# semchan/DCT_Pruning

Measured on AMD Instinct MI355X. Metric: feature-map DCT+score throughput, higher is better.
Workload: dtype f32; 1 GPU; resnet_50 hooked feature maps (49 tensors, 22720 maps/sample: 56x56 x1344, 28x28 x3200, 14x14 x9472, 7x7 x8704), batch 256, limit=steps; global_batch=256, launch_mode=one launch per tile shape, units_rank0=49

## Files before the change

### dct_pruning_amd/csrc/api.hip

```cpp
#include <hip/hip_runtime.h>
#include <stdint.h>

#include <initializer_list>
#include <mutex>

#include "../../include/dctscore.h"
#include "dcts_internal.h"
#include "grid_caps.h"
#include "rect.h"
#ifdef DCTS_FUSED_STAMPS
#include "split_common.hpp"
#endif

using namespace dctsi;

namespace {

struct TensorView {
  const float* x;
  int64_t N, C_total, H, W, strideN, strideC, strideH, strideW;
  int32_t c_begin, c_count;
  bool pad_front_if_odd;

  int pad() const { return (pad_front_if_odd && (H % 2 != 0)) ? 1 : 0; }
// ... 113 lines not shown
    if (algo == DCTS_ALGO_TILE2D || algo == DCTS_ALGO_FUSED) {
      if (!tile_shape || !aligned16) return kUnsupported;
      if (algo == DCTS_ALGO_TILE2D) return {HP == 224 ? Family::Tile2d : Family::Tile2g, DCTS_OK};
      return {has_fused2(HP) ? Family::Fused2 : Family::Fused, DCTS_OK};
    }
    return {Family::Direct, DCTS_OK};
  }
  const bool split_ok = tile_shape && aligned16;
  if (algo == DCTS_ALGO_SPLIT && !split_ok) return kUnsupported;
  if (algo == DCTS_ALGO_AUTO || algo == DCTS_ALGO_FUSED || algo == DCTS_ALGO_PIPE || algo == DCTS_ALGO_TILE2D) {
    if (tile_shape)
      for (const auto& t : kTileOrder) {
        const Family f = t.fam;
        if ((algo != DCTS_ALGO_AUTO && algo != t.algo) || !serves(f, HP)) continue;
        if (!aligned16 && traits(f).base16) continue;
        if (f == Family::Tile2g && algo == DCTS_ALGO_AUTO && aligned16 && tile2g_loses(HP)) continue;
        return {f, DCTS_OK};
      }
    if (pad == 1 && v.dense_maps() && (algo == DCTS_ALGO_AUTO || algo == DCTS_ALGO_TILE2D) && has_tile2g_pad(HP))
      return {Family::Tile2gPad, DCTS_OK};
    if (algo != DCTS_ALGO_AUTO) return kUnsupported;
  }
  if (split_ok && algo != DCTS_ALGO_DIRECT) return {Family::Split, DCTS_OK};
  return {Family::Direct, DCTS_OK};
}

TileBatch single_batch(const TensorView& v, float* out) { return single_tensor_batch(v.base(), out, v.nmaps(), v.strideC); }

struct BasisSlot {
  uintptr_t lo, hi;
  void* ws;
  void* stream;
  int HP, WP;
};
constexpr int kBasisSlots = 16;
BasisSlot g_basis[kBasisSlots] = {};
int g_basis_next = 0;
std::mutex g_basis_mu;

bool basis_cached(void* ws, void* stream, int HP, int WP) {
  std::lock_guard<std::mutex> lk(g_basis_mu);
  for (const BasisSlot& b : g_basis)
    if (b.hi && b.ws == ws && b.stream == stream && b.HP == HP && b.WP == WP) return true;
  return false;
}
void basis_forget_range(const void* p, size_t bytes) {
  if (!p || !bytes) return;
  const uintptr_t lo = reinterpret_cast<uintptr_t>(p), hi = lo + bytes;
  std::lock_guard<std::mutex> lk(g_basis_mu);
  for (BasisSlot& b : g_basis)
    if (b.hi && b.lo < hi && lo < b.hi) b = BasisSlot{};
}
void basis_forget(void* ws) {
  if (!ws) return;
  const uintptr_t a = reinterpret_cast<uintptr_t>(ws);
  std::lock_guard<std::mutex> lk(g_basis_mu);
  for (BasisSlot& b : g_basis)
    if (b.hi && (b.ws == ws || (b.lo <= a && a < b.hi))) b = BasisSlot{};
}
void basis_remember(void* ws, const void* tables, size_t table_bytes, void* stream, int HP, int WP) {
  const uintptr_t lo = reinterpret_cast<uintptr_t>(tables), hi = lo + table_bytes;
  std::lock_guard<std::mutex> lk(g_basis_mu);
  for (BasisSlot& b : g_basis)
    if (b.hi && (b.ws == ws || (b.lo < hi && lo < b.hi))) b = BasisSlot{};
  g_basis[g_basis_next] = BasisSlot{lo, hi, ws, stream, HP, WP};
  g_basis_next = (g_basis_next + 1) % kBasisSlots;
}

int run(bool store, const TensorView& v, float* out, void* workspace, size_t workspace_bytes, void* stream, int32_t algo,
        bool cache_basis = true) {
  if (const int rc = validate(v, {out}, Checks::All)) return rc;
  const Choice c = choose(v, algo, store, v.aligned16());
  if (c.err) return c.err;
  const int HP = (int)v.HP(), WP = (int)v.WP(), pad = v.pad();
  const MapGeom g = map_geom(v);
  hipStream_t st = reinterpret_cast<hipStream_t>(stream);
  switch (c.fam) {
    case Family::Rect: return dispatch_rect(rect_geom(v), out, store ? 1 : 0, st);
    case Family::CodeletDma: return dispatch_codelet_dma(HP, g, out, st);
    case Family::Codelet: return dispatch_codelet(store ? 1 : 0, HP, WP, pad, g, out, st);
    case Family::Direct: break;
    case Family::Lane: {
      MultiGeom mg;
      for (int i = 0; i < kMultiItems; ++i) mg.it[i] = MultiItem{g, out, 0};
      mg.total_groups = (g.nmaps + 63) / 64;
      mg.count = 1;
      return dispatch_lane(HP, mg, st);
    }
    case Family::Split: {
      const SplitWs sws = split_ws(g.nmaps, HP);
      if (!workspace || workspace_bytes < sws.total) return DCTS_E_WORKSPACE;
      if (reinterpret_cast<uintptr_t>(workspace) & 15) return DCTS_E_ALIGN;
      basis_forget_range(workspace, sws.total);
      return dispatch_split(HP, g, out, workspace, st);
    }
    default: {
      if (!store) return traits(c.fam).batch(HP, single_batch(v, out), st);
      const long long tile_bytes = (long long)HP * WP * 4;
      const long long ws_maps = workspace ? (long long)(workspace_bytes / (size_t)tile_bytes) : 0;
      if (ws_maps < 1 || (reinterpret_cast<uintptr_t>(workspace) & 15)) return DCTS_E_WORKSPACE;
      float* scratch = reinterpret_cast<float*>(workspace);
      basis_forget_range(workspace, workspace_bytes);
      switch (c.fam) {
        case Family::Tile2d: return dispatch_tile2d_coeff(HP, v.base(), g.nmaps, out, scratch, ws_maps, st);
        case Family::Tile2g: return dispatch_tile2g_coeff(HP, v.base(), g.nmaps, out, scratch, ws_maps, st);
        case Family::Fused2: return dispatch_fused2_coeff(HP, v.base(), g.nmaps, out, scratch, ws_maps, st);
        default: return dispatch_fused_coeff(HP, v.base(), g.nmaps, out, scratch, ws_maps, st);
      }
    }
  }

  const DirectWs ws = direct_ws(g.nmaps, HP, WP);
  if (!workspace) return ws.total ? DCTS_E_WORKSPACE : DCTS_E_NULL;
  if (workspace_bytes < ws.total) return DCTS_E_WORKSPACE;
  char* wsp = reinterpret_cast<char*>(workspace);
  float* CHt = reinterpret_cast<float*>(wsp + ws.off_ch);
  float* CWt = reinterpret_cast<float*>(wsp + ws.off_cw);
  float* T = reinterpret_cast<float*>(wsp + ws.off_t);
  int rc_tables = 0;
  if (!cache_basis || !basis_cached(workspace, stream, HP, WP)) {
    basis_forget_range(workspace, ws.total);
    const int rc = launch_basis(CHt, HP, CWt, WP, st);
    if (cache_basis && rc == hipSuccess) basis_remember(workspace, wsp + ws.off_ch, ws.off_t - ws.off_ch, stream, HP, WP);
    if (!cache_basis) rc_tables = rc;
  } else {
    basis_forget_range(wsp + ws.off_t, ws.total - ws.off_t);
  }
  const int rc = dispatch_direct(store ? 1 : 0, pad, g, ws.grid, CHt, CWt, T, out, st);
  return rc ? rc : rc_tables;
}

int coeff_algo(const TensorView& v) {
  const int HP = (int)v.HP();
  if (v.pad() != 0 || !v.dense_square() || (v.strideN * 4) % 16 != 0 || !v.aligned16()) return DCTS_ALGO_AUTO;
  if (serves(Family::Tile2d, HP) || serves(Family::Tile2g, HP)) return DCTS_ALGO_TILE2D;
  if (serves(Family::Fused, HP) || serves(Family::Fused2, HP)) return DCTS_ALGO_FUSED;
  return DCTS_ALGO_AUTO;
}

template <class F>
int for_chunks(int64_t N, int64_t c_count, long long chunk, bool whole_samples, F f) {
  if (whole_samples) {
    const int64_t ns = chunk / c_count;
    for (int64_t n0 = 0; n0 < N; n0 += ns)
      if (const int rc = f(n0, (N - n0) < ns ? (N - n0) : ns, (int64_t)0, c_count)) return rc;
    return DCTS_OK;
  }
  for (int64_t n = 0; n < N; ++n)
    for (int64_t c0 = 0; c0 < c_count; c0 += chunk)
      if (const int rc = f(n, (int64_t)1, c0, (c_count - c0) < chunk ? (c_count - c0) : chunk)) return rc;
  return DCTS_OK;
}

struct CoeffWs {
  long long chunk;
  float* coeff;
  void* inner;
  size_t inner_bytes;
};
CoeffWs coeff_ws(void* workspace, size_t workspace_bytes, long long chunk, size_t tile) {
  const size_t off_inner = align_up((size_t)chunk * tile, 256);
  char* wsp = reinterpret_cast<char*>(workspace);
  return CoeffWs{chunk, reinterpret_cast<float*>(wsp), wsp + off_inner, workspace_bytes - off_inner};
}

template <class Reduce>
int coeff_chunks(const TensorView& v, const CoeffWs& w, bool whole_samples, int algo, void* workspace, size_t workspace_bytes,
                 void* stream, Reduce reduce) {
  basis_forget(workspace);
  basis_forget_range(workspace, workspace_bytes);
// ... 296 lines not shown

int dcts_has_half_kernel(int64_t H, int64_t W) { return has_half(H, W) ? 1 : 0; }

int dcts_energy_typed(const void* x, int32_t dtype, int64_t N, int64_t C_total, int64_t H, int64_t W, int64_t strideN,
                      int64_t strideC, int64_t strideH, int64_t strideW, int32_t c_begin, int32_t c_count,
                      int32_t pad_front_if_odd, float* out_nc, void* workspace, size_t workspace_bytes, void* stream) {
  if (dtype == DCTS_DTYPE_F32)
    return dcts_energy_f32(reinterpret_cast<const float*>(x), N, C_total, H, W, strideN, strideC, strideH, strideW, c_begin,
                           c_count, pad_front_if_odd, out_nc, workspace, workspace_bytes, stream);
  if (!is_half_dtype(dtype)) return DCTS_E_UNSUPPORTED;
  const TensorView v = view_of(x, N, C_total, H, W, strideN, strideC, strideH, strideW, c_begin, c_count, pad_front_if_odd);
  if (const int rc = validate(v, {out_nc}, Checks::All, true, elem_mask(dtype))) return rc;
  hipStream_t st = reinterpret_cast<hipStream_t>(stream);
  const uint16_t* xh = reinterpret_cast<const uint16_t*>(x);
  if (has_half(H, W) && v.pad() == 0 && strideH == W)
    return dispatch_half((int)H, dtype, HalfGeom{xh, v.nmaps(), strideN, strideC, c_count, c_begin, v.contiguous() ? 1 : 0}, out_nc, st);

  if (!workspace) return DCTS_E_WORKSPACE;
  if (reinterpret_cast<uintptr_t>(workspace) & 15) return DCTS_E_ALIGN;
  const size_t map = (size_t)H * W * 4;
  const size_t inner_bytes = align_up(dcts_workspace_bytes(N, c_count, H, W), 256);
  if (workspace_bytes < inner_bytes + map) return DCTS_E_WORKSPACE;
  long long chunk = (long long)((workspace_bytes - inner_bytes) / map);
  if ((size_t)chunk * map > kHalfStageCap && kHalfStageCap >= map) chunk = (long long)(kHalfStageCap / map);
  float* stage = reinterpret_cast<float*>(reinterpret_cast<char*>(workspace) + inner_bytes);
  void* inner = inner_bytes ? workspace : nullptr;
  basis_forget_range(stage, (size_t)chunk * map);
  return for_chunks(N, c_count, chunk, chunk >= c_count, [&](int64_t n0, int64_t ns, int64_t c0, int64_t nc) -> int {
    const HalfGeom g{xh + n0 * strideN, ns * nc, strideN, strideC, (int)nc, (int)(c_begin + c0), (ns == 1 || strideN == nc * strideC) ? 1 : 0};
    if (const int rc = launch_upcast_half(dtype, g, (int)H, (int)W, strideH, stage, st)) return rc;
    const TensorView s{stage, ns, nc, H, W, nc * H * W, H * W, W, 1, 0, (int32_t)nc, pad_front_if_odd != 0};
    return run(false, s, out_nc + n0 * c_count + c0, inner, inner_bytes, stream, DCTS_ALGO_AUTO);
  });
}

int dcts_has_nhwc_kernel(int64_t H, int64_t W) { return has_nhwc(H, W) ? 1 : 0; }

size_t dcts_nhwc_workspace_bytes(int32_t, int64_t, int64_t, int64_t, int64_t) { return 0; }

int dcts_energy_nhwc(const void* x, int32_t dtype, int64_t N, int64_t C_total, int64_t H, int64_t W, int64_t strideN,
                     int64_t strideH, int64_t strideW, int32_t c_begin, int32_t c_count, float* out_nc, void*, size_t, void* stream) {
  if (dtype != DCTS_DTYPE_F32 && !is_half_dtype(dtype)) return DCTS_E_UNSUPPORTED;
  const TensorView v = view_of(x, N, C_total, H, W, strideN, 1, strideH, strideW, c_begin, c_count, 0);
  if (const int rc = validate(v, {out_nc}, Checks::All, true, elem_mask(dtype), true)) return rc;
  if (!has_nhwc(H, W)) return DCTS_E_UNSUPPORTED;
  return dispatch_nhwc((int)H, dtype, NhwcGeom{x, N, strideN, strideH, strideW, c_begin, c_count}, out_nc, reinterpret_cast<hipStream_t>(stream));
}

int dcts_batch_sum_f32(const float* energy_nc, int64_t N, int64_t C_count, float* out_c,
                       void* stream) {
  if (!energy_nc || !out_c) return DCTS_E_NULL;
  if (N <= 0 || C_count <= 0) return DCTS_E_SHAPE;
  return launch_batch_sum(energy_nc, N, C_count, out_c, reinterpret_cast<hipStream_t>(stream));
}

int dcts_running_mean_update_f32(const float* energy_nc, int64_t N, int64_t C_count,
                                 float* feature_result, float total_before, void* stream) {
  if (!energy_nc || !feature_result) return DCTS_E_NULL;
  if (N <= 0 || C_count <= 0) return DCTS_E_SHAPE;
  return launch_running_mean(energy_nc, N, C_count, feature_result, total_before, reinterpret_cast<hipStream_t>(stream));
}

int dcts_energy_multi_f32(const dcts_tensor_item* items, int32_t count, int64_t H, int64_t W,
                          int32_t pad_front_if_odd, void* workspace, size_t workspace_bytes, void* stream) {
  if (!items) return DCTS_E_NULL;
  if (count <= 0 || H <= 0 || W <= 0) return DCTS_E_SHAPE;
  for (int32_t i = 0; i < count; ++i)
    if (const int rc = validate(view_of(items[i], H, W, pad_front_if_odd), {items[i].out_nc}, Checks::Align)) return rc;
  const TensorView v0 = view_of(items[0], H, W, pad_front_if_odd);
  const int HP = (int)v0.HP(), WP = (int)v0.WP(), pad = v0.pad();
  hipStream_t st = reinterpret_cast<hipStream_t>(stream);
  if (has_codelet(HP, WP)) {
    const int G = codelet_group_size(HP);
    for (int32_t i0 = 0; i0 < count; i0 += kMultiItems) {
      const int n = (count - i0) < kMultiItems ? (count - i0) : kMultiItems;
      MultiGeom mg;
      long long groups = 0;
      for (int i = 0; i < n; ++i) {
        mg.it[i].g = map_geom(view_of(items[i0 + i], H, W, pad_front_if_odd));
        mg.it[i].out = items[i0 + i].out_nc;
        mg.it[i].group_begin = groups;
        groups += (mg.it[i].g.nmaps + G - 1) / G;
      }
      for (int i = n; i < kMultiItems; ++i) mg.it[i] = mg.it[0];
      mg.total_groups = groups;
      mg.count = n;
      const int rc = dispatch_codelet_multi(HP, pad, mg, st);
      if (rc) return rc;
    }
    return DCTS_OK;
  }
  TileBatch tb;
  Family fam = Family::Direct;
  int nb = 0;
  auto flush = [&]() -> int {
    if (!nb) return DCTS_OK;
    for (int i = nb; i < kTileItems; ++i) {
      tb.x[i] = tb.x[0];
      tb.out[i] = tb.out[0];
      tb.begin[i + 1] = tb.begin[nb];
    }
    tb.map_elems = H * W;
    tb.total = tb.begin[nb];
    tb.count = nb;
    nb = 0;
    return traits(fam).batch(HP, tb, st);
  };
  for (int32_t i = 0; i < count; ++i) {
    const TensorView v = view_of(items[i], H, W, pad_front_if_odd);
    const Choice c = choose(v, DCTS_ALGO_AUTO, false, true);
    if (!c.err && traits(c.fam).batch && (v.aligned16() || !traits(c.fam).base16)) {
      if (nb == 0) tb.begin[0] = 0;
      fam = c.fam;
      tb.x[nb] = v.base();
      tb.out[nb] = items[i].out_nc;
      tb.begin[nb + 1] = tb.begin[nb] + v.nmaps();
      if (++nb == kTileItems) {
        const int rc = flush();
        if (rc) return rc;
      }
      continue;
    }
    const int rc = run(false, v, items[i].out_nc, workspace, workspace_bytes, stream, DCTS_ALGO_AUTO);
    if (rc) return rc;
  }
  return flush();
}

int dcts_energy_mixed_f32(const dcts_shaped_item* items, int32_t count, void* workspace, size_t workspace_bytes,
                          void* stream) {
  if (!items) return DCTS_E_NULL;
  if (count <= 0) return DCTS_E_SHAPE;
  hipStream_t st = reinterpret_cast<hipStream_t>(stream);
  for (int32_t i = 0; i < count; ++i)
    if (const int rc = validate(view_of(items[i]), {items[i].t.out_nc}, Checks::Align)) return rc;
  auto eligible = [&](const dcts_shaped_item& it) {
    return it.H == it.W && mixed_has((int)it.H) && !(it.pad_front_if_odd && (it.H % 2 != 0));
  };
  MixedGeom mg;
  int n = 0;
  long long groups = 0;
  auto flush = [&]() -> int {
    if (!n) return DCTS_OK;
    for (int i = n; i < kMixedItems; ++i) mg.it[i] = mg.it[0];
    mg.total_groups = groups;
    mg.count = n;
    n = 0;
    groups = 0;
    return dispatch_codelet_mixed(mg, st);
  };
  for (int32_t i = 0; i < count; ++i) {
    if (!eligible(items[i])) continue;
    mg.it[n].g = map_geom(view_of(items[i]));
    mg.it[n].out = items[i].t.out_nc;
    mg.it[n].group_begin = groups;
    const int G = 64 / (int)items[i].H;
    groups += (mg.it[n].g.nmaps + G - 1) / G;
    if (++n == kMixedItems) {
      const int rc = flush();
      if (rc) return rc;
    }
  }
  int rc = flush();
  if (rc) return rc;
  dcts_tensor_item buf[64];
  for (int32_t i = 0; i < count; ++i) {
    if (eligible(items[i])) continue;
    bool seen = false;
    for (int32_t k = 0; k < i && !seen; ++k)
      seen = !eligible(items[k]) && items[k].H == items[i].H && items[k].W == items[i].W &&
// ... 58 lines not shown
```

### dct_pruning_amd/csrc/codelet.hip

```cpp
#include <hip/hip_runtime.h>
#include <stdint.h>

#include "../../include/dctscore.h"
#include "codelet_schedule.hpp"
#include "codelet_sizes.h"
#include "dct_codelets.hpp"
#include "dcts_internal.h"
#include "grid_caps.h"
#include "split_roles.hpp"

using namespace dctsi;

namespace {

template <int O0, int O1, int O2, int O3>
__device__ __forceinline__ void lds_write_addtid4(unsigned base, float a, float b, float c, float d) {
  static_assert(O3 < 65536 && O0 >= 0, "16-bit offset field");
  asm volatile(
      "s_mov_b32 m0, %0\n\ts_nop 0\n\t"
      "ds_write_addtid_b32 %1 offset:%5\n\tds_write_addtid_b32 %2 offset:%6\n\t"
      "ds_write_addtid_b32 %3 offset:%7\n\tds_write_addtid_b32 %4 offset:%8"
      :
      : "s"(base), "v"(a), "v"(b), "v"(c), "v"(d), "n"(O0), "n"(O1), "n"(O2), "n"(O3)
      : "memory", "m0");
// ... 29 lines not shown
      dcts::static_for<HP>([&](auto i) DCTS_LAMBDA_INLINE { xr[decltype(i)::value] = 0.f; });
    }
  }
  float y[HP];
  dcts::Dct2<HP>::run(xr, y);
  y[0] *= dcts::kInvSqrt2;
  if constexpr (G == 1 && HP % 4 == 0) {
    if (act1) {
      const unsigned base = (unsigned)__builtin_amdgcn_readfirstlane((int)(unsigned)(unsigned long long)(lds_ptr)my);
      dcts::static_for<HP / 4>([&](auto i) DCTS_LAMBDA_INLINE {
        constexpr int k0 = 4 * decltype(i)::value;
        lds_write_addtid4<k0 * S * 4, (k0 + 1) * S * 4, (k0 + 2) * S * 4, (k0 + 3) * S * 4>(base, y[k0], y[k0 + 1], y[k0 + 2], y[k0 + 3]);
      });
    }
  } else
  if (act1) {
    float* dst = my + g1 * MAP_LDS + c;
    dcts::static_for<HP>([&](auto i) DCTS_LAMBDA_INLINE {
      constexpr int kk = decltype(i)::value;
      dst[kk * S] = y[kk];
    });
  }
  wave_fence();

  float z[WP], w[WP];
  {
    const float* src = my + (act2 ? g2 : 0) * MAP_LDS + (act2 ? k : 0) * S;
    dcts::static_for<WP>([&](auto i) DCTS_LAMBDA_INLINE {
      constexpr int cc = decltype(i)::value;
      z[cc] = src[cc];
    });
  }
  dcts::Dct2<WP>::run(z, w);
  w[0] *= dcts::kInvSqrt2;
  const long long m2 = grp * G + g2;
  if constexpr (STORE_COEFF) {
    if (act2 && m2 < g.nmaps) {
      constexpr float sc = float(2.0 / dcts::cx_sqrt(double(HP) * double(WP)));
      float* o = out + (m2 * HP + k) * WP;
      dcts::static_for<WP>([&](auto i) DCTS_LAMBDA_INLINE {
        constexpr int l = decltype(i)::value;
        o[l] = w[l] * sc;
      });
    }
  } else {
    float e = 0.f;
    dcts::static_for<WP>([&](auto i) DCTS_LAMBDA_INLINE {
      constexpr int l = decltype(i)::value;
      e = fmaf(w[l], w[l], e);
    });
    if (!act2) e = 0.f;
    DCTS_MAP_SUM(HP, e, k)
    if (act2 && k == 0 && m2 < g.nmaps) {
      constexpr float sc = float(4.0 / (double(HP) * double(WP)));
      out[m2] = e * sc;
    }
  }
  wave_fence();
}

template <int HP, int WP, int PAD, bool STORE_COEFF>
__global__ __launch_bounds__((64 * CodeletCfg<HP>::WAVES)) void k_energy_codelet(
    MapGeom g, float* __restrict__ out) {
  using Cfg = CodeletCfg<HP>;
  constexpr int G = Cfg::G, WAVES = Cfg::WAVES;
  __shared__ float slab[WAVES][Cfg::WAVE_LDS];

  const int lane = threadIdx.x & 63;
  const int wave = threadIdx.x >> 6;
  float* my = slab[wave];

  const int g1 = lane / WP, c = lane - g1 * WP;
  const int g2 = lane / HP, k = lane - g2 * HP;
  const bool act1 = g1 < G, act2 = g2 < G;

  const long long ngroups = (g.nmaps + G - 1) / G;
  const long long wave_gid = (long long)blockIdx.x * WAVES + wave;
  const long long nwaves = (long long)gridDim.x * WAVES;

  for (long long grp = wave_gid; grp < ngroups; grp += nwaves)
    codelet_group<HP, WP, PAD, STORE_COEFF>(g, out, grp, my, g1, c, g2, k, act1, act2);
}

template <int HP, int WP, int PAD>
__global__ __launch_bounds__((64 * CodeletCfg<HP>::WAVES)) void k_energy_codelet_multi(MultiGeom mg) {
  using Cfg = CodeletCfg<HP>;
  constexpr int G = Cfg::G, WAVES = Cfg::WAVES;
  __shared__ float slab[WAVES][Cfg::WAVE_LDS];

  const int lane = threadIdx.x & 63;
  const int wave = threadIdx.x >> 6;
  float* my = slab[wave];
  const int g1 = lane / WP, c = lane - g1 * WP;
  const int g2 = lane / HP, k = lane - g2 * HP;
  const bool act1 = g1 < G, act2 = g2 < G;

  const long long wave_gid = (long long)blockIdx.x * WAVES + wave;
  const long long nwaves = (long long)gridDim.x * WAVES;
  int t = 0;
  for (long long grp = wave_gid; grp < mg.total_groups; grp += nwaves) {
    while (t + 1 < mg.count && grp >= mg.it[t + 1].group_begin) ++t;
    t = __builtin_amdgcn_readfirstlane(t);
    const MultiItem& item = mg.it[t];
    codelet_group<HP, WP, PAD, false>(item.g, item.out, grp - item.group_begin, my, g1, c, g2, k, act1, act2);
  }
}

constexpr int mixed_slab_floats() {
  int m = 0;
#define DCTS_CASE(N) \
  if (CodeletCfg<N>::WAVE_LDS > m) m = CodeletCfg<N>::WAVE_LDS;
  DCTS_MIXED_SIZES(DCTS_CASE)
#undef DCTS_CASE
  return m;
}

template <int E>
__device__ __forceinline__ void mixed_group(const MultiItem& item, long long grp, float* my, int lane) {
  using Cfg = CodeletCfg<E>;
  const int g1 = lane / E, c = lane - g1 * E;
  const bool act = g1 < Cfg::G;
  codelet_group<E, E, 0, false>(item.g, item.out, grp, my, g1, c, g1, c, act, act);
}

__global__ __launch_bounds__((64 * kMixedWaves)) void k_energy_codelet_mixed(MixedGeom mg) {
  __shared__ float slab[kMixedWaves][mixed_slab_floats()];
  const int lane = threadIdx.x & 63;
  const int wave = threadIdx.x >> 6;
  float* my = slab[wave];
  const long long wave_gid = (long long)blockIdx.x * kMixedWaves + wave;
  const long long nwaves = (long long)gridDim.x * kMixedWaves;
  int t = 0;
  for (long long grp = wave_gid; grp < mg.total_groups; grp += nwaves) {
    while (t + 1 < mg.count && grp >= mg.it[t + 1].group_begin) ++t;
    t = __builtin_amdgcn_readfirstlane(t);
    const MultiItem& item = mg.it[t];
    const long long local = grp - item.group_begin;
    switch (__builtin_amdgcn_readfirstlane(item.g.H)) {
#define DCTS_CASE(N)                          \
  case N:                                     \
    mixed_group<N>(item, local, my, lane);    \
    break;
      DCTS_MIXED_SIZES(DCTS_CASE)
#undef DCTS_CASE
      default:
        break;
    }
  }
}

template <int N>
struct LaneCfg {
  static constexpr int NN = N * N;
  static constexpr int G = kLaneMultiGroup;
  static constexpr int SLAB = (G * NN + 3) / 4 * 4;
  static constexpr int ITERS = (G * NN / 4 + 63) / 64;
  static constexpr int WAVES = kLaneMultiWaves;
  static_assert(NN % 2 == 1, "lane stride must be odd (bank conflicts) - even tiles use the codelet kernel");
};

struct LaneGroup {
  const float* src;
  float* out;
  long long m0;
  int nm;
  int dense;
  int item;
};

template <int N>
__device__ __forceinline__ void lane_stage(const LaneGroup& gr, lds_ptr my, int lane) {
  using Cfg = LaneCfg<N>;
  if (!gr.dense) return;
  const int nfl = gr.nm * Cfg::NN, nq = nfl >> 2, rem = nfl & 3;
  const unsigned long long sa = reinterpret_cast<unsigned long long>(gr.src);
  const unsigned long long src = ((unsigned long long)__builtin_amdgcn_readfirstlane((int)(sa >> 32)) << 32) |
                                 (unsigned)__builtin_amdgcn_readfirstlane((int)sa);
  const unsigned base = (unsigned)__builtin_amdgcn_readfirstlane((int)(unsigned)(unsigned long long)my);
#pragma unroll
  for (int it = 0; it < Cfg::ITERS; ++it) {
    const int q = it * 64 + lane;
    if (q < nq) {
      const unsigned dst = base + it * 1024;
      const unsigned off = (unsigned)q * 16u;
      asm volatile("s_mov_b32 m0, %0\n\ts_nop 0\n\tglobal_load_lds_dwordx4 %1, %2"
                   :
                   : "s"(dst), "v"(off), "s"(src)
                   : "memory", "m0");
    }
  }
  if (lane < rem) my[4 * nq + lane] = gr.src[4 * nq + lane];
}

template <int N>
__device__ __forceinline__ void lane_compute(const MapGeom& g, const LaneGroup& gr, lds_ptr my, int lane,
                                             float (&v)[N * N]) {
  constexpr int NN = N * N;
  const bool act = lane < gr.nm;
  if (gr.dense) {
    lds_cptr p = my + (act ? lane : 0) * NN;
    dcts::static_for<NN>([&](auto i) DCTS_LAMBDA_INLINE { v[decltype(i)::value] = p[decltype(i)::value]; });
  } else {
    const float* p = map_base(g, gr.m0 + (act ? lane : 0));
    dcts::static_for<NN>([&](auto i) DCTS_LAMBDA_INLINE { v[decltype(i)::value] = p[decltype(i)::value]; });
  }
}

template <int N>
__device__ __forceinline__ float lane_energy(float (&v)[N * N]) {
  dcts::static_for<N>([&](auto ic) DCTS_LAMBDA_INLINE {
    constexpr int c = decltype(ic)::value;
    float in[N], o[N];
    dcts::static_for<N>([&](auto ir) DCTS_LAMBDA_INLINE { in[decltype(ir)::value] = v[decltype(ir)::value * N + c]; });
    dcts::Dct2<N>::run(in, o);
    o[0] *= dcts::kInvSqrt2;
    dcts::static_for<N>([&](auto ir) DCTS_LAMBDA_INLINE { v[decltype(ir)::value * N + c] = o[decltype(ir)::value]; });
  });
  float e = 0.f;
  dcts::static_for<N>([&](auto ir) DCTS_LAMBDA_INLINE {
    constexpr int r = decltype(ir)::value;
    float in[N], o[N];
    dcts::static_for<N>([&](auto ic) DCTS_LAMBDA_INLINE { in[decltype(ic)::value] = v[r * N + decltype(ic)::value]; });
    dcts::Dct2<N>::run(in, o);
    o[0] *= dcts::kInvSqrt2;
    dcts::static_for<N>([&](auto ic) DCTS_LAMBDA_INLINE { e = fmaf(o[decltype(ic)::value], o[decltype(ic)::value], e); });
  });
  constexpr float sc = float(4.0 / (double(N) * double(N)));
  return e * sc;
}

__device__ __forceinline__ LaneGroup lane_group_of(const MapGeom& g, float* out, long long grp, int nn, int item) {
  LaneGroup gr;
  gr.m0 = grp * 64;
  const long long left = g.nmaps - gr.m0;
  gr.nm = (int)(left < 64 ? left : 64);
  gr.src = g.x + (long long)g.c_begin * g.strideC + gr.m0 * nn;
  gr.dense = (g.contiguous && g.strideC == nn && ((reinterpret_cast<unsigned long long>(gr.src) & 15) == 0)) ? 1 : 0;
  gr.out = out + gr.m0;
  gr.item = item;
  return gr;
}

template <int N>
__global__ __launch_bounds__((64 * LaneCfg<N>::WAVES)) void k_energy_lane_multi(MultiGeom mg) {
  using Cfg = LaneCfg<N>;
  __shared__ __attribute__((aligned(16))) float slab[Cfg::WAVES][Cfg::SLAB];
  const int lane = threadIdx.x & 63;
  const int wave = threadIdx.x >> 6;
  const lds_ptr my = (lds_ptr)slab[wave];
  const long long wave_gid = (long long)blockIdx.x * Cfg::WAVES + wave;
  const long long nwaves = (long long)gridDim.x * Cfg::WAVES;
  int t = 0;
  auto locate = [&](long long grp) DCTS_LAMBDA_INLINE {
    while (t + 1 < mg.count && grp >= mg.it[t + 1].group_begin) ++t;
    t = __builtin_amdgcn_readfirstlane(t);
    return lane_group_of(mg.it[t].g, mg.it[t].out, grp - mg.it[t].group_begin, Cfg::NN, t);
  };
  if (wave_gid >= mg.total_groups) return;
  LaneGroup cur = locate(wave_gid);
  lane_stage<N>(cur, my, lane);
  for (long long grp = wave_gid; grp < mg.total_groups; grp += nwaves) {
    asm volatile("s_waitcnt vmcnt(0)" ::: "memory");
    float v[Cfg::NN];
    lane_compute<N>(mg.it[cur.item].g, cur, my, lane, v);
    asm volatile("s_waitcnt lgkmcnt(0)" ::: "memory");
    const LaneGroup done = cur;
    if (grp + nwaves < mg.total_groups) {
      cur = locate(grp + nwaves);
      lane_stage<N>(cur, my, lane);
    }
    const float e = lane_energy<N>(v);
    if (lane < done.nm) done.out[lane] = e;
  }
}

template <int N>
__global__ __launch_bounds__((64 * CodeletCfg<N>::WAVES)) void k_energy_codelet_dma(
    MapGeom g, float* __restrict__ out) {
  using Cfg = CodeletCfg<N>;
  constexpr int G = Cfg::G, S = Cfg::S, MAP_LDS = Cfg::MAP_LDS, WAVES = Cfg::WAVES;
  constexpr int NN = N * N;
  constexpr int QPG = G * NN / 4;
  constexpr int DMA_IT = (QPG + 63) / 64;
  constexpr int SLAB = ((Cfg::WAVE_LDS > DMA_IT * 256 ? Cfg::WAVE_LDS : DMA_IT * 256) + 3) / 4 * 4;
  static_assert((G * NN) % 4 == 0, "group must be a whole number of 16-byte quads");
  __shared__ __attribute__((aligned(16))) float slab[WAVES][SLAB];

  const int lane = threadIdx.x & 63;
  const int wave = threadIdx.x >> 6;
  float* my = slab[wave];
  const int g1 = lane / N, c = lane - g1 * N;
  const bool act = g1 < G;

  const long long ngroups = (g.nmaps + G - 1) / G;
  const long long wave_gid = (long long)blockIdx.x * WAVES + wave;
  const long long nwaves = (long long)gridDim.x * WAVES;
  const float* x0 = g.x + (long long)g.c_begin * g.strideC;

  auto prefetch = [&](long long grp) DCTS_LAMBDA_INLINE {
    const long long m0 = grp * G;
    const long long left = g.nmaps - m0;
    const int nq = (int)((left < G ? left : G) * (NN / 4));
    const float* src = x0 + m0 * NN;
#pragma unroll
    for (int it = 0; it < DMA_IT; ++it) {
      const int q = it * 64 + lane;
      if (q < nq)
        __builtin_amdgcn_global_load_lds((const __attribute__((address_space(1))) void*)(src + 4 * q),
                                         (__attribute__((address_space(3))) void*)(my + it * 256), 16, 0, 0);
    }
  };

  if (wave_gid < ngroups) prefetch(wave_gid);
  for (long long grp = wave_gid; grp < ngroups; grp += nwaves) {
    asm volatile("s_waitcnt vmcnt(0)" ::: "memory");
    const long long m1 = grp * G + g1;
    const bool valid = act && m1 < g.nmaps;
    float xr[N], y[N];
    {
      const float* src = my + (valid ? g1 * NN + c : 0);
      dcts::static_for<N>([&](auto i) DCTS_LAMBDA_INLINE {
        constexpr int r = decltype(i)::value;
        xr[r] = src[r * N];
      });
      if (!valid) dcts::static_for<N>([&](auto i) DCTS_LAMBDA_INLINE { xr[decltype(i)::value] = 0.f; });
    }
    dcts::Dct2<N>::run(xr, y);
    y[0] *= dcts::kInvSqrt2;
    __builtin_amdgcn_fence(__ATOMIC_RELEASE, "wavefront");
    __builtin_amdgcn_wave_barrier();
    if (act) {
      float* dst = my + g1 * MAP_LDS + c;
      dcts::static_for<N>([&](auto i) DCTS_LAMBDA_INLINE {
        constexpr int kk = decltype(i)::value;
        dst[kk * S] = y[kk];
      });
    }
    wave_fence();
    float z[N], w[N];
    {
      const float* src = my + (act ? g1 : 0) * MAP_LDS + (act ? c : 0) * S;
      dcts::static_for<N>([&](auto i) DCTS_LAMBDA_INLINE {
        constexpr int cc = decltype(i)::value;
        z[cc] = src[cc];
      });
    }
    asm volatile("s_waitcnt lgkmcnt(0)" ::: "memory");
    __builtin_amdgcn_fence(__ATOMIC_RELEASE, "wavefront");
    __builtin_amdgcn_wave_barrier();
    if (grp + nwaves < ngroups) prefetch(grp + nwaves);
    dcts::Dct2<N>::run(z, w);
    w[0] *= dcts::kInvSqrt2;
    float e = 0.f;
    dcts::static_for<N>([&](auto i) DCTS_LAMBDA_INLINE {
      constexpr int l = decltype(i)::value;
      e = fmaf(w[l], w[l], e);
    });
    if (!act) e = 0.f;
    DCTS_MAP_SUM(N, e, c)
    if (valid && c == 0) {
      constexpr float sc = float(4.0 / (double(N) * double(N)));
      out[m1] = e * sc;
    }
  }
}

template <int HP, int WP, int PAD, bool STORE>
int launch_codelet(const MapGeom& g, float* out, hipStream_t st) {
  using Cfg = CodeletCfg<HP>;
  const long long ngroups = (g.nmaps + Cfg::G - 1) / Cfg::G;
  hipLaunchKernelGGL((k_energy_codelet<HP, WP, PAD, STORE>), dim3(codelet_grid<HP>(ngroups)), dim3(64 * Cfg::WAVES), 0, st, g, out);
  return (int)hipGetLastError();
}

template <int N>
int launch_codelet_dma(const MapGeom& g, float* out, hipStream_t st) {
  using Cfg = CodeletCfg<N>;
  if constexpr ((Cfg::G * N * N) % 4 != 0) {
    return DCTS_E_UNSUPPORTED;
  } else {
    const long long ngroups = (g.nmaps + Cfg::G - 1) / Cfg::G;
    const long long cap = (long long)num_cus() * blocks_per_cu<k_energy_codelet_dma<N>, Cfg::WAVES>();
    hipLaunchKernelGGL((k_energy_codelet_dma<N>), dim3(grid_blocks(ngroups, Cfg::WAVES, cap)), dim3(64 * Cfg::WAVES), 0, st, g, out);
    return (int)hipGetLastError();
  }
}

template <int HP, int WP, int PAD>
int launch_codelet_multi(const MultiGeom& mg, hipStream_t st) {
  hipLaunchKernelGGL((k_energy_codelet_multi<HP, WP, PAD>), dim3(codelet_grid<HP>(mg.total_groups)), dim3(64 * CodeletCfg<HP>::WAVES),
                     0, st, mg);
  return (int)hipGetLastError();
}

template <int N>
int launch_lane(const MultiGeom& mg, hipStream_t st) {
  using Cfg = LaneCfg<N>;
  const long long cap = (long long)num_cus() * blocks_per_cu<k_energy_lane_multi<N>, Cfg::WAVES>();
  hipLaunchKernelGGL((k_energy_lane_multi<N>), dim3(grid_blocks(mg.total_groups, Cfg::WAVES, cap)), dim3(64 * Cfg::WAVES), 0, st, mg);
  return (int)hipGetLastError();
}

}

namespace dctsi {

int codelet_group_size(int HP) {
  if (has_lane_kernel(HP)) return 64;
#define DCTS_CASE(N) \
  if (HP == N) return CodeletCfg<N>::G;
  DCTS_CODELET_SIZES(DCTS_CASE)
#undef DCTS_CASE
  return 0;
}

int dispatch_codelet_dma(int N, const MapGeom& g, float* out, hipStream_t st) {
#define DCTS_CASE(N_) \
  case N_:            \
    return launch_codelet_dma<N_>(g, out, st);
  switch (N) {
    DCTS_CODELET_SIZES(DCTS_CASE)
    default:
      return DCTS_E_UNSUPPORTED;
  }
#undef DCTS_CASE
}

int dispatch_codelet(int store, int HP, int WP, int pad, const MapGeom& g, float* out, hipStream_t st) {
  if (HP != WP) return DCTS_E_UNSUPPORTED;
  return switch_codelet_size(HP, pad, [&](auto n, auto p) {
    constexpr int N = decltype(n)::value, PAD = decltype(p)::value;
    return store ? launch_codelet<N, N, PAD, true>(g, out, st) : launch_codelet<N, N, PAD, false>(g, out, st);
  });
}

int dispatch_codelet_mixed(const MixedGeom& mg, hipStream_t st) {
  const long long cap = (long long)num_cus() * blocks_per_cu<k_energy_codelet_mixed, kMixedWaves>();
  hipLaunchKernelGGL(k_energy_codelet_mixed, dim3(grid_blocks(mg.total_groups, kMixedWaves, cap)), dim3(64 * kMixedWaves), 0, st, mg);
  return (int)hipGetLastError();
}

int dispatch_lane(int n, const MultiGeom& mg, hipStream_t st) {
  switch (n) {
    case 7:
      return launch_lane<7>(mg, st);
    case 9:
      return launch_lane<9>(mg, st);
    default:
      return DCTS_E_UNSUPPORTED;
  }
}

int dispatch_codelet_multi(int HP, int pad, const MultiGeom& mg, hipStream_t st) {
  if (has_lane_kernel(HP) && pad == 0) return dispatch_lane(HP, mg, st);
  return switch_codelet_size(HP, pad, [&](auto n, auto p) {
    return launch_codelet_multi<decltype(n)::value, decltype(n)::value, decltype(p)::value>(mg, st);
  });
}

}
```

### dct_pruning_amd/csrc/dcts_internal.h

```cpp
#pragma once
#include <hip/hip_runtime.h>
#include <stddef.h>
#include <stdint.h>

#include "codelet_sizes.h"

struct dcts_update_desc;

namespace dctsi {

struct MapGeom {
  const float* x;
  long long nmaps;
  long long strideN;
  long long strideC;
  long long strideH;
  int c_count;
  int c_begin;
  int H, W;
  int contiguous;
};

template <class Geom>
__device__ __forceinline__ auto map_base(const Geom& g, long long m) -> decltype(g.x) {
  if (g.contiguous) return g.x + (long long)g.c_begin * g.strideC + m * g.strideC;
  const long long n = m / g.c_count;
  const long long j = m - n * g.c_count;
  return g.x + n * g.strideN + (g.c_begin + j) * g.strideC;
}

constexpr int kMultiItems = 32;
struct MultiItem {
  MapGeom g;
  float* out;
  long long group_begin;
};
struct MultiGeom {
  MultiItem it[kMultiItems];
  long long total_groups;
  int count;
};

constexpr int kMixedItems = 48;
struct MixedGeom {
  MultiItem it[kMixedItems];
  long long total_groups;
  int count;
};
#define DCTS_MIXED_SIZES(X) X(2) X(4) X(8) X(16) X(32)
constexpr bool mixed_has(int e) {
#define DCTS_CASE(N) \
  if (e == N) return true;
  DCTS_MIXED_SIZES(DCTS_CASE)
#undef DCTS_CASE
  return false;
}

constexpr int kTileItems = 32;
struct TileBatch {
  const float* x[kTileItems];
  float* out[kTileItems];
  long long begin[kTileItems + 1];
  long long map_elems;
  long long total;
  int count;
};

inline TileBatch single_tensor_batch(const float* x, float* out, long long nmaps, long long map_elems) {
  TileBatch tb;
  for (int i = 0; i < kTileItems; ++i) {
    tb.x[i] = x;
    tb.out[i] = out;
    tb.begin[i] = 0;
  }
  tb.begin[1] = tb.begin[kTileItems] = nmaps;
  tb.map_elems = map_elems;
  tb.total = nmaps;
  tb.count = 1;
  return tb;
}

inline int num_cus() {
  static const int n = [] {
    int dev = 0, cu = 0;
    if (hipGetDevice(&dev) != hipSuccess ||
        hipDeviceGetAttribute(&cu, hipDeviceAttributeMultiprocessorCount, dev) != hipSuccess || cu < 1)
      cu = 256;
    return cu;
  }();
  return n;
}

inline size_t align_up(size_t v, size_t a) { return (v + a - 1) / a * a; }

inline bool has_codelet(long long HP, long long WP) {
  if (HP != WP) return false;
#define DCTS_CASE(N) \
  if (HP == N) return true;
  DCTS_CODELET_SIZES(DCTS_CASE)
#undef DCTS_CASE
  return false;
}

constexpr bool has_lane_kernel(int n) { return n == 7 || n == 9; }

inline bool has_split(long long HP, long long WP) {
  if (HP != WP) return false;
#define DCTS_CASE(N_, M_, L_) \
  if (HP == N_) return true;
  DCTS_SPLIT_TABLE(DCTS_CASE)
#undef DCTS_CASE
  return false;
}

inline bool has_fused(long long N) {
#define DCTS_CASE(N_, M_, L_) \
  if (N == N_) return true;
  DCTS_FUSED_TABLE(DCTS_CASE)
#undef DCTS_CASE
  return false;
}

inline bool has_fused2(long long N) {
#define DCTS_CASE(N_, M_, L_) \
// ... 128 lines not shown
```

Baseline: 3720 Mmaps/s.

## Precompute dense per-item descriptors and use 32-bit windowed group indexing in multi kernels

The host now precomputes per-item dense descriptors (base pointer, ragged tail, density flag) and a padded int32 group_begin table. Launches are split into windows so device loops can use 32-bit indices, and item lookup uses an unrolled branchless walk. The codelet multi kernel gains a dense fast path that resolves the next item during the LDS exchange. The lane kernel prefetches the next group descriptor before computing, hiding scalar address math and 64-bit arithmetic. The cost is a larger kernel argument struct and more code paths.

```diff
diff --git a/dct_pruning_amd/csrc/api.hip b/dct_pruning_amd/csrc/api.hip
--- a/dct_pruning_amd/csrc/api.hip
+++ b/dct_pruning_amd/csrc/api.hip
@@ -219,10 +219,8 @@
     case Family::Direct: break;
     case Family::Lane: {
       MultiGeom mg;
-      for (int i = 0; i < kMultiItems; ++i) mg.it[i] = MultiItem{g, out, 0};
-      mg.total_groups = (g.nmaps + 63) / 64;
-      mg.count = 1;
-      return dispatch_lane(HP, mg, st);
+      mg.it[0] = MultiItem{g, out, 0};
+      return multi_launch(mg, 1, (g.nmaps + 63) / 64, 64, true, [&](const MultiGeom& w) { return dispatch_lane(HP, w, st); });
     }
     case Family::Split: {
       const SplitWs sws = split_ws(g.nmaps, HP);
@@ -685,10 +683,8 @@
         mg.it[i].group_begin = groups;
         groups += (mg.it[i].g.nmaps + G - 1) / G;
       }
-      for (int i = n; i < kMultiItems; ++i) mg.it[i] = mg.it[0];
-      mg.total_groups = groups;
-      mg.count = n;
-      const int rc = dispatch_codelet_multi(HP, pad, mg, st);
+      const int rc = multi_launch(mg, n, groups, G, has_lane_kernel(HP) && pad == 0,
+                                  [&](const MultiGeom& w) { return dispatch_codelet_multi(HP, pad, w, st); });
       if (rc) return rc;
     }
     return DCTS_OK;
diff --git a/dct_pruning_amd/csrc/codelet.hip b/dct_pruning_amd/csrc/codelet.hip
--- a/dct_pruning_amd/csrc/codelet.hip
+++ b/dct_pruning_amd/csrc/codelet.hip
@@ -135,27 +135,147 @@
     codelet_group<HP, WP, PAD, STORE_COEFF>(g, out, grp, my, g1, c, g2, k, act1, act2);
 }
 
+
+__device__ __forceinline__ int multi_walk(const MultiGeom& mg, int t, int grp) {
+  for (;;) {
+    const int* b = &mg.group_begin[t + 1];
+    int n = 0;
+#pragma unroll
+    for (int i = 0; i < kMultiWalk; ++i) n = grp >= b[i] ? i + 1 : n;
+    t += n;
+    if (n < kMultiWalk) return t;
+  }
+}
+
+struct MultiCur {
+  MultiDense d;
+  float* out;
+  int begin;
+  __device__ __forceinline__ long long local(int grp) const { return d.local0 + (grp - begin); }
+  __device__ __forceinline__ int maps(long long loc, int G) const { return loc == d.ragged_local ? d.tail : G; }
+};
+__device__ __forceinline__ MultiCur multi_fetch(const MultiGeom& mg, int t) { return MultiCur{mg.d[t], mg.it[t].out, mg.group_begin[t]}; }
+
+template <int HP, int WP, int PAD, class Between>
+__device__ __forceinline__ void codelet_group_dense(const float* gbase, unsigned off, bool ld, float* __restrict__ o, bool st, float* my,
+                                                    int g1, int c, int g2, int k, bool act1, bool act2, Between&& between) {
+  using Cfg = CodeletCfg<HP>;
+  constexpr int G = Cfg::G, S = Cfg::S, MAP_LDS = Cfg::MAP_LDS;
+  constexpr int W = WP - PAD;
+  float xr[HP];
+  const float* p = gbase + off;
+  if constexpr (PAD == 0) {
+    dcts::static_for<HP>([&](auto i) DCTS_LAMBDA_INLINE {
+      constexpr int r = decltype(i)::value;
+      xr[r] = p[r * W];
+    });
+  } else {
+    if (ld) {
+      dcts::static_for<HP>([&](auto i) DCTS_LAMBDA_INLINE {
+        constexpr int r = decltype(i)::value;
+        if constexpr (r < PAD)
+          xr[r] = 0.f;
+        else
+          xr[r] = p[(r - PAD) * W];
+      });
+    } else {
+      dcts::static_for<HP>([&](auto i) DCTS_LAMBDA_INLINE { xr[decltype(i)::value] = 0.f; });
+    }
+  }
+  float y[HP];
+  dcts::Dct2<HP>::run(xr, y);
+  y[0] *= dcts::kInvSqrt2;
+  if constexpr (G == 1 && HP % 4 == 0) {
+    if (act1) {
+      const unsigned base = (unsigned)__builtin_amdgcn_readfirstlane((int)(unsigned)(unsigned long long)(lds_ptr)my);
+      dcts::static_for<HP / 4>([&](auto i) DCTS_LAMBDA_INLINE {
+        constexpr int k0 = 4 * decltype(i)::value;
+        lds_write_addtid4<k0 * S * 4, (k0 + 1) * S * 4, (k0 + 2) * S * 4, (k0 + 3) * S * 4>(base, y[k0], y[k0 + 1], y[k0 + 2], y[k0 + 3]);
+      });
+    }
+  } else
+  if (act1) {
+    float* dst = my + g1 * MAP_LDS + c;
+    dcts::static_for<HP>([&](auto i) DCTS_LAMBDA_INLINE {
+      constexpr int kk = decltype(i)::value;
+      dst[kk * S] = y[kk];
+    });
+  }
+  between();
+  wave_fence();
+
+  float z[WP], w[WP];
+  {
+    const float* src = my + (act2 ? g2 : 0) * MAP_LDS + (act2 ? k : 0) * S;
+    dcts::static_for<WP>([&](auto i) DCTS_LAMBDA_INLINE {
+      constexpr int cc = decltype(i)::value;
+      z[cc] = src[cc];
+    });
+  }
+  dcts::Dct2<WP>::run(z, w);
+  w[0] *= dcts::kInvSqrt2;
+  float e = 0.f;
+  dcts::static_for<WP>([&](auto i) DCTS_LAMBDA_INLINE {
+    constexpr int l = decltype(i)::value;
+    e = fmaf(w[l], w[l], e);
+  });
+  if (!act2) e = 0.f;
+  DCTS_MAP_SUM(HP, e, k)
+  if (st) {
+    constexpr float sc = float(4.0 / (double(HP) * double(WP)));
+    o[g2] = e * sc;
+  }
+  wave_fence();
+}
+
 template <int HP, int WP, int PAD>
 __global__ __launch_bounds__((64 * CodeletCfg<HP>::WAVES)) void k_energy_codelet_multi(MultiGeom mg) {
   using Cfg = CodeletCfg<HP>;
   constexpr int G = Cfg::G, WAVES = Cfg::WAVES;
+  constexpr int MAP = (HP - PAD) * (WP - PAD);
   __shared__ float slab[WAVES][Cfg::WAVE_LDS];
 
   const int lane = threadIdx.x & 63;
-  const int wave = threadIdx.x >> 6;
+  const int wave = __builtin_amdgcn_readfirstlane(threadIdx.x >> 6);
   float* my = slab[wave];
   const int g1 = lane / WP, c = lane - g1 * WP;
   const int g2 = lane / HP, k = lane - g2 * HP;
   const bool act1 = g1 < G, act2 = g2 < G;
-
-  const long long wave_gid = (long long)blockIdx.x * WAVES + wave;
-  const long long nwaves = (long long)gridDim.x * WAVES;
-  int t = 0;
-  for (long long grp = wave_gid; grp < mg.total_groups; grp += nwaves) {
-    while (t + 1 < mg.count && grp >= mg.it[t + 1].group_begin) ++t;
-    t = __builtin_amdgcn_readfirstlane(t);
-    const MultiItem& item = mg.it[t];
-    codelet_group<HP, WP, PAD, false>(item.g, item.out, grp - item.group_begin, my, g1, c, g2, k, act1, act2);
+  const bool ld_full = act1 && c >= PAD, st_full = act2 && k == 0;
+  const unsigned off_full = ld_full ? (unsigned)(g1 * MAP + c - PAD) : 0u;
+
+  const int wave_gid = (int)blockIdx.x * WAVES + wave;
+  const int nwaves = (int)gridDim.x * WAVES;
+  if (wave_gid >= mg.groups) return;
+  int t = multi_walk(mg, 0, wave_gid);
+  MultiCur cur = multi_fetch(mg, t);
+  for (int grp = wave_gid; grp < mg.groups; grp += nwaves) {
+    const long long local = cur.local(grp);
+    const int tc = t;
+    MultiCur nxt = cur;
+    auto resolve_next = [&]() DCTS_LAMBDA_INLINE {
+      if (grp + nwaves < mg.groups) {
+        t = multi_walk(mg, t, grp + nwaves);
+        nxt = multi_fetch(mg, t);
+      }
+    };
+    if (cur.d.dense) {
+      bool ld = ld_full, st = st_full;
+      unsigned off = off_full;
+      if constexpr (G > 1) {
+        const int nm = cur.maps(local, G);
+        ld = ld_full && g1 < nm;
+        st = st_full && g2 < nm;
+        off = ld ? off_full : 0u;
+      }
+      codelet_group_dense<HP, WP, PAD>(cur.d.base + local * (G * MAP), off, ld, cur.out + local * G, st, my, g1, c, g2, k, act1, act2,
+                                       resolve_next);
+    } else {
+      resolve_next();
+      const MultiItem& item = mg.it[tc];
+      codelet_group<HP, WP, PAD, false>(item.g, item.out, local, my, g1, c, g2, k, act1, act2);
+    }
+    cur = nxt;
   }
 }
 
@@ -282,48 +402,44 @@
   return e * sc;
 }
 
-__device__ __forceinline__ LaneGroup lane_group_of(const MapGeom& g, float* out, long long grp, int nn, int item) {
-  LaneGroup gr;
-  gr.m0 = grp * 64;
-  const long long left = g.nmaps - gr.m0;
-  gr.nm = (int)(left < 64 ? left : 64);
-  gr.src = g.x + (long long)g.c_begin * g.strideC + gr.m0 * nn;
-  gr.dense = (g.contiguous && g.strideC == nn && ((reinterpret_cast<unsigned long long>(gr.src) & 15) == 0)) ? 1 : 0;
-  gr.out = out + gr.m0;
-  gr.item = item;
-  return gr;
-}
-
 template <int N>
 __global__ __launch_bounds__((64 * LaneCfg<N>::WAVES)) void k_energy_lane_multi(MultiGeom mg) {
   using Cfg = LaneCfg<N>;
   __shared__ __attribute__((aligned(16))) float slab[Cfg::WAVES][Cfg::SLAB];
   const int lane = threadIdx.x & 63;
-  const int wave = threadIdx.x >> 6;
+  const int wave = __builtin_amdgcn_readfirstlane(threadIdx.x >> 6);
   const lds_ptr my = (lds_ptr)slab[wave];
-  const long long wave_gid = (long long)blockIdx.x * Cfg::WAVES + wave;
-  const long long nwaves = (long long)gridDim.x * Cfg::WAVES;
+  const int wave_gid = (int)blockIdx.x * Cfg::WAVES + wave;
+  const int nwaves = (int)gridDim.x * Cfg::WAVES;
   int t = 0;
-  auto locate = [&](long long grp) DCTS_LAMBDA_INLINE {
-    while (t + 1 < mg.count && grp >= mg.it[t + 1].group_begin) ++t;
-    t = __builtin_amdgcn_readfirstlane(t);
-    return lane_group_of(mg.it[t].g, mg.it[t].out, grp - mg.it[t].group_begin, Cfg::NN, t);
+  auto locate = [&](int grp) DCTS_LAMBDA_INLINE {
+    t = multi_walk(mg, t, grp);
+    const MultiCur it = multi_fetch(mg, t);
+    const long long local = it.local(grp);
+    LaneGroup gr;
+    gr.m0 = local * Cfg::G;
+    gr.nm = it.maps(local, Cfg::G);
+    gr.src = it.d.base + gr.m0 * Cfg::NN;
+    gr.dense = it.d.dense;
+    gr.out = it.out + gr.m0;
+    gr.item = t;
+    return gr;
   };
-  if (wave_gid >= mg.total_groups) return;
+  if (wave_gid >= mg.groups) return;
   LaneGroup cur = locate(wave_gid);
   lane_stage<N>(cur, my, lane);
-  for (long long grp = wave_gid; grp < mg.total_groups; grp += nwaves) {
+  for (int grp = wave_gid; grp < mg.groups; grp += nwaves) {
+    const bool more = grp + nwaves < mg.groups;
+    LaneGroup nxt = cur;
+    if (more) nxt = locate(grp + nwaves);
     asm volatile("s_waitcnt vmcnt(0)" ::: "memory");
     float v[Cfg::NN];
     lane_compute<N>(mg.it[cur.item].g, cur, my, lane, v);
     asm volatile("s_waitcnt lgkmcnt(0)" ::: "memory");
-    const LaneGroup done = cur;
-    if (grp + nwaves < mg.total_groups) {
-      cur = locate(grp + nwaves);
-      lane_stage<N>(cur, my, lane);
-    }
+    if (more) lane_stage<N>(nxt, my, lane);
     const float e = lane_energy<N>(v);
-    if (lane < done.nm) done.out[lane] = e;
+    if (lane < cur.nm) cur.out[lane] = e;
+    cur = nxt;
   }
 }
 
@@ -441,7 +557,7 @@
 
 template <int HP, int WP, int PAD>
 int launch_codelet_multi(const MultiGeom& mg, hipStream_t st) {
-  hipLaunchKernelGGL((k_energy_codelet_multi<HP, WP, PAD>), dim3(codelet_grid<HP>(mg.total_groups)), dim3(64 * CodeletCfg<HP>::WAVES),
+  hipLaunchKernelGGL((k_energy_codelet_multi<HP, WP, PAD>), dim3(codelet_grid<HP>(mg.groups)), dim3(64 * CodeletCfg<HP>::WAVES),
                      0, st, mg);
   return (int)hipGetLastError();
 }
@@ -450,7 +566,7 @@
 int launch_lane(const MultiGeom& mg, hipStream_t st) {
   using Cfg = LaneCfg<N>;
   const long long cap = (long long)num_cus() * blocks_per_cu<k_energy_lane_multi<N>, Cfg::WAVES>();
-  hipLaunchKernelGGL((k_energy_lane_multi<N>), dim3(grid_blocks(mg.total_groups, Cfg::WAVES, cap)), dim3(64 * Cfg::WAVES), 0, st, mg);
+  hipLaunchKernelGGL((k_energy_lane_multi<N>), dim3(grid_blocks(mg.groups, Cfg::WAVES, cap)), dim3(64 * Cfg::WAVES), 0, st, mg);
   return (int)hipGetLastError();
 }
 
diff --git a/dct_pruning_amd/csrc/dcts_internal.h b/dct_pruning_amd/csrc/dcts_internal.h
--- a/dct_pruning_amd/csrc/dcts_internal.h
+++ b/dct_pruning_amd/csrc/dcts_internal.h
@@ -35,11 +35,51 @@
   float* out;
   long long group_begin;
 };
+struct MultiDense {
+  const float* base;
+  long long ragged_local;
+  long long local0;
+  int tail;
+  int dense;
+};
+constexpr int kMultiWalk = 4;
+constexpr long long kMultiWindow = 1LL << 30;
 struct MultiGeom {
+  int group_begin[kMultiItems + kMultiWalk];
+  int groups;
+  int count;
+  MultiDense d[kMultiItems];
   MultiItem it[kMultiItems];
   long long total_groups;
-  int count;
-};
+};
+static_assert(sizeof(MultiGeom) <= 4096, "kernel arguments");
+
+inline void multi_window(MultiGeom& mg, int n, long long total, long long g0, int G, bool lane16) {
+  for (int i = n; i < kMultiItems; ++i) mg.it[i] = mg.it[0];
+  for (int i = 0; i < kMultiItems; ++i) {
+    const MapGeom& g = mg.it[i].g;
+    const float* base = g.x + (long long)g.c_begin * g.strideC;
+    const bool dense = g.contiguous && g.strideC == (long long)g.H * g.W && (!lane16 || (reinterpret_cast<uintptr_t>(base) & 15) == 0);
+    const int tail = (int)(g.nmaps % G);
+    const long long begin = mg.it[i].group_begin;
+    mg.d[i] = MultiDense{base, tail ? g.nmaps / G : -1, g0 > begin ? g0 - begin : 0, tail, dense ? 1 : 0};
+  }
+  for (int i = 0; i < kMultiItems + kMultiWalk; ++i) {
+    const long long rel = i < n ? mg.it[i].group_begin - g0 : 0x7fffffffLL;
+    mg.group_begin[i] = (int)(rel < 0 ? 0 : (rel > 0x7fffffffLL ? 0x7fffffffLL : rel));
+  }
+  mg.groups = (int)(total - g0 < kMultiWindow ? total - g0 : kMultiWindow);
+  mg.count = n;
+  mg.total_groups = total;
+}
+template <class Launch>
+int multi_launch(MultiGeom& mg, int n, long long total, int G, bool lane16, Launch&& launch) {
+  for (long long g0 = 0; g0 < total; g0 += kMultiWindow) {
+    multi_window(mg, n, total, g0, G, lane16);
+    if (const int rc = launch(mg)) return rc;
+  }
+  return 0;
+}
 
 constexpr int kMixedItems = 48;
 struct MixedGeom {
```

Measured after the change: 3742 Mmaps/s (median of 6 runs). About the same (+0.6%).
